# audiohacking/fp8-mps-metal

Measured on NVIDIA B200. Metric: FP8 _scaled_mm TFLOPS & M=1 GEMV/cast HBM GB/s as % roofline vs CPU ref, higher is better.
Workload: dtype f32

## Files before the change

fp8-mps-metal_b200/csrc/fp8_gemm_tcgen05.cu:

```cuda
#include <cuda.h>
#include <cstdio>
#include <mutex>
#include <type_traits>

#include "fp8_mm.cuh"
#include "fp8_async.cuh"

namespace fp8b {

constexpr int kBM = 128;
constexpr int kBK = 128;
constexpr int kUmmaK = 32;
#ifndef FP8B_EPI_WARPS
#define FP8B_EPI_WARPS 4
#endif
constexpr int kNumEpiWarps = FP8B_EPI_WARPS;
constexpr int kEpiColSplits = kNumEpiWarps / 4;
enum { kStDirect = 0, kStPeers = 1, kStTma = 2, kStWide = 3 };
template <int MODE> constexpr bool is_push() { return MODE == kStTma || MODE == kStWide; }
constexpr int kMaxDst = 8;
template <int MODE> constexpr int gemm_threads() { return 64 + 32 * kNumEpiWarps + (is_push<MODE>() ? 32 : 0); }

constexpr int kStoreBoxBytes = 128 * 128;
#ifndef FP8B_TMA_SLOTS
// ... 125 lines not shown
    uint32_t r;
    asm volatile("mov.u32 %0, %%cluster_ctarank;" : "=r"(r));
    return r;
}
__device__ __forceinline__ void cluster_sync_all() {
    asm volatile("barrier.cluster.arrive.release.aligned;" ::: "memory");
    asm volatile("barrier.cluster.wait.acquire.aligned;" ::: "memory");
}
__device__ __forceinline__ void cluster_sync_relaxed() {
    asm volatile("barrier.cluster.arrive.relaxed.aligned;" ::: "memory");
    asm volatile("barrier.cluster.wait.aligned;" ::: "memory");
}
__device__ __forceinline__ void tma_load_2d_2sm(uint32_t smem_dst, const CUtensorMap* m, uint32_t bar, int c0, int c1) {
    asm volatile("cp.async.bulk.tensor.2d.cta_group::2.shared::cluster.global.mbarrier::complete_tx::bytes [%0], [%1, {%3, %4}], [%2];"
                 :: "r"(smem_dst), "l"(reinterpret_cast<uint64_t>(m)), "r"(bar & kPeerBitMask), "r"(c0), "r"(c1) : "memory");
}
__device__ __forceinline__ void mbar_arrive_leader(uint32_t bar) {
    asm volatile("mbarrier.arrive.shared::cluster.b64 _, [%0];" :: "r"(bar & kPeerBitMask) : "memory");
}
__device__ __forceinline__ void tmem_alloc_2sm(uint32_t smem_dst, uint32_t ncols) {
    asm volatile("tcgen05.alloc.cta_group::2.sync.aligned.shared::cta.b32 [%0], %1;" :: "r"(smem_dst), "r"(ncols) : "memory");
}
__device__ __forceinline__ void tmem_relinquish_2sm() {
    asm volatile("tcgen05.relinquish_alloc_permit.cta_group::2.sync.aligned;" ::: "memory");
}
__device__ __forceinline__ void tmem_dealloc_2sm(uint32_t taddr, uint32_t ncols) {
    asm volatile("tcgen05.dealloc.cta_group::2.sync.aligned.b32 %0, %1;" :: "r"(taddr), "r"(ncols) : "memory");
}
__device__ __forceinline__ void umma_f8_2sm(uint32_t tmem_d, uint64_t adesc, uint64_t bdesc, uint32_t idesc, uint32_t accumulate) {
    asm volatile("{\n\t.reg .pred p;\n\tsetp.ne.b32 p, %4, 0;\n\t"
                 "tcgen05.mma.cta_group::2.kind::f8f6f4 [%0], %1, %2, %3, p;\n\t}"
                 :: "r"(tmem_d), "l"(adesc), "l"(bdesc), "r"(idesc), "r"(accumulate) : "memory");
}
__device__ __forceinline__ void umma_commit_2sm(uint32_t bar) {
    asm volatile("tcgen05.commit.cta_group::2.mbarrier::arrive::one.shared::cluster.multicast::cluster.b64 [%0], %1;"
                 :: "r"(bar), "h"((uint16_t)3) : "memory");
}

__device__ __forceinline__ bool elect_one() {
    uint32_t pred;
    asm volatile("{\n\t.reg .pred p;\n\telect.sync _|p, 0xFFFFFFFF;\n\tselp.u32 %0, 1, 0, p;\n\t}" : "=r"(pred));
    return pred != 0;
}

__device__ __forceinline__ uint64_t make_smem_desc(uint32_t smem_addr) {
    uint64_t d = 0;
    d |= (uint64_t)((smem_addr & 0x3FFFF) >> 4);
    d |= (uint64_t)1 << 16;
    d |= (uint64_t)(1024 >> 4) << 32;
    d |= (uint64_t)1 << 46;
    d |= (uint64_t)2 << 61;
    return d;
}

__host__ __device__ constexpr uint32_t make_idesc(int m, int n) {
    return (1u << 4) | ((uint32_t)(n >> 3) << 17) | ((uint32_t)(m >> 4) << 24);
}

__device__ __forceinline__ void stg_v4(void* p, uint32_t a, uint32_t b, uint32_t c, uint32_t d, int mc) {
    if (mc)
        asm volatile("multimem.st.weak.global.v4.f32 [%0], {%1,%2,%3,%4};"
                     :: "l"(p), "f"(__uint_as_float(a)), "f"(__uint_as_float(b)), "f"(__uint_as_float(c)),
                        "f"(__uint_as_float(d)) : "memory");
    else
        asm volatile("st.global.v4.u32 [%0], {%1,%2,%3,%4};" :: "l"(p), "r"(a), "r"(b), "r"(c), "r"(d) : "memory");
}

__device__ __forceinline__ void sts_v4(uint32_t addr, uint32_t a, uint32_t b, uint32_t c, uint32_t d) {
    asm volatile("st.shared.v4.u32 [%0], {%1,%2,%3,%4};" :: "r"(addr), "r"(a), "r"(b), "r"(c), "r"(d) : "memory");
}
__device__ __forceinline__ void lds_v4(uint32_t addr, uint32_t& a, uint32_t& b, uint32_t& c, uint32_t& d) {
    asm volatile("ld.shared.v4.u32 {%0,%1,%2,%3}, [%4];" : "=r"(a), "=r"(b), "=r"(c), "=r"(d) : "r"(addr) : "memory");
}

constexpr int kRasterGroup = 8;
struct TileCoord { int m_blk; int n0; int width; };
__device__ __forceinline__ TileCoord decode_tile(const GemmParams& p, int t, int bn) {
    TileCoord c;
    int tt = t, half = -1;
    if (t >= p.full_tiles) {
        const int u = t - p.full_tiles;
        tt = p.full_tiles + (u >> 1);
        half = u & 1;
    }
    int n_blk;
    if (p.raster_n == 2) {
        const int per_band = kRasterGroup * p.num_n_blocks;
        const int band = tt / per_band, r = tt - band * per_band;
        const int m0 = band * kRasterGroup;
        const int rows = min(kRasterGroup, p.num_m_blocks - m0);
        c.m_blk = m0 + r % rows;
        n_blk = r / rows;
    }
    else if (p.raster_n) { n_blk = tt % p.num_n_blocks; c.m_blk = tt / p.num_n_blocks; }
    else { c.m_blk = tt % p.num_m_blocks; n_blk = tt / p.num_m_blocks; }
    c.width = half < 0 ? bn : bn >> 1;
    c.n0 = n_blk * bn + (half > 0 ? c.width : 0);
    return c;
}

template <bool SBV, bool BIAS, bool SR>
__device__ __forceinline__ void epi_math32(const uint32_t (&r)[32], float sa, float sb0, float sr, const float (&sbv)[32],
                                           const float (&bv)[32], float (&v)[32]) {
#pragma unroll
    for (int j = 0; j < 32; ++j) {
        float x = __fmul_rn(__uint_as_float(r[j]), sa);
        x = __fmul_rn(x, SBV ? sbv[j] : sb0);
        if (BIAS) x = __fadd_rn(x, bv[j]);
        if (SR) x = __fmul_rn(x, sr);
        v[j] = x;
    }
}
__device__ __forceinline__ bool any_nan32(const uint32_t (&r)[32]) {
    float s0 = 0.0f, s1 = 0.0f, s2 = 0.0f, s3 = 0.0f;
#pragma unroll
    for (int j = 0; j < 32; j += 4) {
        s0 += __uint_as_float(r[j]); s1 += __uint_as_float(r[j + 1]);
        s2 += __uint_as_float(r[j + 2]); s3 += __uint_as_float(r[j + 3]);
    }
    const float s = (s0 + s1) + (s2 + s3);
    return s != s;
}

static __device__ __noinline__ void fix_nan_chunk(uint32_t* r, const uint8_t* a_row, const uint8_t* b_rows, int K, int n_left,
                                                  int a_fmt, int b_fmt) {
    for (int j = 0; j < 32 && j < n_left; ++j) {
        const float a = __uint_as_float(r[j]);
        if (a != a) r[j] = __float_as_uint(slow_dot_fmt(a_row, b_rows + (size_t)j * K, K, a_fmt, b_fmt));
    }
}
// ... 25 lines not shown
                    const float4 t = b4[j];
                    bv[4 * j] = t.x; bv[4 * j + 1] = t.y; bv[4 * j + 2] = t.z; bv[4 * j + 3] = t.w;
                }
            } else {
                const uint4* b4 = reinterpret_cast<const uint4*>(reinterpret_cast<const uint16_t*>(e.bias) + n0);
#pragma unroll
                for (int j = 0; j < 4; ++j) {
                    const uint4 t = b4[j];
                    const uint32_t w[4] = {t.x, t.y, t.z, t.w};
#pragma unroll
                    for (int i = 0; i < 4; ++i) {
                        if (e.bias_dtype == FP8B_BF16) {
                            bv[8 * j + 2 * i] = __uint_as_float(w[i] << 16);
                            bv[8 * j + 2 * i + 1] = __uint_as_float(w[i] & 0xFFFF0000u);
                        } else {
                            const float2 f = __half22float2(*reinterpret_cast<const __half2*>(&w[i]));
                            bv[8 * j + 2 * i] = f.x; bv[8 * j + 2 * i + 1] = f.y;
                        }
                    }
                }
            }
        }
    } else {
#pragma unroll
        for (int j = 0; j < 32; ++j) {
            const int n = n0 + j;
            const bool ok = n < N;
            sbv[j] = (e.sb_stride && ok) ? e.sb[n] : 0.0f;
            bv[j] = (e.bias && ok) ? epi_bias(e, n) : 0.0f;
        }
    }
}

template <int BN, int CG, int MODE = kStDirect>
__global__ void __launch_bounds__(gemm_threads<MODE>(), 1)
fp8_gemm_tcgen05_kernel(const __grid_constant__ CUtensorMap tmap_a,
                        const __grid_constant__ CUtensorMap tmap_b,
                        const __grid_constant__ typename StoreMapsOf<MODE>::type smaps,
                        const GemmParams p)
{
    using Cfg = GemmCfg<BN, CG, MODE>;
    constexpr bool PEERS = MODE == kStPeers;
#ifdef FP8B_PROFILE
    long long* const dbg = PEERS ? nullptr : p.aux;
#endif
    constexpr int kTileM = kBM * CG;
    const uint32_t cta_rank = (CG == 2) ? cluster_ctarank() : 0u;
    const bool is_leader = cta_rank == 0;
    const int worker = (CG == 2) ? (int)(blockIdx.x >> 1) : (int)blockIdx.x;
    const int num_workers = (CG == 2) ? (int)(gridDim.x >> 1) : (int)gridDim.x;
    extern __shared__ uint8_t gemm_smem_raw[];
    uint8_t* smem = reinterpret_cast<uint8_t*>((reinterpret_cast<uintptr_t>(gemm_smem_raw) + 1023) & ~(uintptr_t)1023);
    uint8_t* bar_mem = smem + Cfg::kOffBar;
    const uint32_t smem_base = smem_u32(smem);
    const uint32_t bar_base = smem_u32(bar_mem);
    auto full_bar = [&](int s) { return bar_base + 8u * s; };
    auto empty_bar = [&](int s) { return bar_base + 8u * (Cfg::kStages + s); };
    auto tfull_bar = [&](int a) { return bar_base + 8u * (2 * Cfg::kStages + a); };
    auto tempty_bar = [&](int a) { return bar_base + 8u * (2 * Cfg::kStages + 2 + a); };
    auto sfull_bar = [&](int s) { return bar_base + 8u * (2 * Cfg::kStages + 4 + s); };
    auto sfree_bar = [&](int s) { return bar_base + 8u * (2 * Cfg::kStages + 4 + Cfg::kStoreSlots + s); };
    volatile uint32_t* tmem_slot =
        reinterpret_cast<volatile uint32_t*>(bar_mem + 8 * (2 * Cfg::kStages + 4 + 2 * Cfg::kStoreSlots));
    const uint32_t stage_base = smem_base + Cfg::kOffStaging;

    const int warp = __shfl_sync(0xFFFFFFFFu, (int)(threadIdx.x >> 5), 0);
    const int lane = threadIdx.x & 31;
#ifdef FP8B_PROFILE
    if (dbg && blockIdx.x == 0 && threadIdx.x == 0) dbg[7] = clock64();
#endif

    pdl_launch_dependents();

    if (warp == kWarpTma && lane == 0) {
        tma_prefetch_desc(&tmap_a);
        tma_prefetch_desc(&tmap_b);
    }
    if (warp == kWarpMma && lane == 0) {
        for (int s = 0; s < Cfg::kStages; ++s) { mbar_init(full_bar(s), 1); mbar_init(empty_bar(s), 1); }
        for (int a = 0; a < 2; ++a) { mbar_init(tfull_bar(a), 1); mbar_init(tempty_bar(a), kNumEpiWarps * CG); }
        if (is_push<MODE>())
            for (int s = 0; s < Cfg::kStoreSlots; ++s) { mbar_init(sfull_bar(s), kNumEpiWarps); mbar_init(sfree_bar(s), 1); }
        fence_mbar_init();
        fence_proxy_async_smem();
    }
    if (warp == kWarpEpi0) {
        if (CG == 2) { tmem_alloc_2sm(smem_u32(const_cast<uint32_t*>(tmem_slot)), Cfg::kTmemCols); tmem_relinquish_2sm(); }
        else { tmem_alloc(smem_u32(const_cast<uint32_t*>(tmem_slot)), Cfg::kTmemCols); tmem_relinquish(); }
    }
    tc_fence_before();
    if (CG == 2) cluster_sync_all();
    else __syncthreads();
    tc_fence_after();
    const uint32_t tmem_base = *tmem_slot;
    pdl_wait();

    const int num_tiles = p.num_work;

    if (warp == kWarpTma) {
        {
            const bool elected = elect_one();
            int stage = 0; uint32_t phase = 0;
#ifdef FP8B_PROFILE
            int issued = 0;
#endif
            for (int tile = worker; tile < num_tiles; tile += num_workers) {
                const TileCoord tc = decode_tile(p, tile, BN);
                const int m_idx = tc.m_blk * kTileM + (int)cta_rank * kBM;
                const int n_idx = tc.n0 + (int)cta_rank * (tc.width / CG);
                for (int kb = 0; kb < p.num_k_blocks; ++kb) {
                    mbar_wait(empty_bar(stage), phase ^ 1);
                    const uint32_t a_dst = smem_base + stage * Cfg::kStageBytes;
                    if (elected) {
#ifdef FP8B_PROFILE
                        if ((p.debug & 32) && issued >= Cfg::kStages) {
                            if (is_leader) mbar_arrive(full_bar(stage));
                        } else
#endif
                        if (CG == 2) {
                            if (is_leader) mbar_arrive_expect_tx(full_bar(stage), (uint32_t)p.stage_tx * CG);
                            tma_load_2d_2sm(a_dst, &tmap_a, full_bar(stage), kb * kBK, m_idx);
                            tma_load_2d_2sm(a_dst + Cfg::kABytes, &tmap_b, full_bar(stage), kb * kBK, n_idx);
                        } else {
                            mbar_arrive_expect_tx(full_bar(stage), (uint32_t)p.stage_tx);
                            tma_load_2d(a_dst, &tmap_a, full_bar(stage), kb * kBK, m_idx);
                            tma_load_2d(a_dst + Cfg::kABytes, &tmap_b, full_bar(stage), kb * kBK, n_idx);
                        }
                    }
                    __syncwarp();
#ifdef FP8B_PROFILE
                    ++issued;
#endif
                    if (++stage == Cfg::kStages) { stage = 0; phase ^= 1; }
                }
            }
        }
    } else if (warp == kWarpMma) {
        if (is_leader) {
            constexpr uint32_t idesc = make_idesc(kTileM, BN);
            const uint32_t idesc_fmt = (((uint32_t)p.debug >> 8) & 1u) << 7 | (((uint32_t)p.debug >> 9) & 1u) << 10;
            const bool elected = elect_one();
            const uint64_t desc_a0 = make_smem_desc(smem_base);
            const uint64_t desc_b0 = make_smem_desc(smem_base + Cfg::kABytes);
            constexpr uint64_t kDescStage = (uint64_t)(Cfg::kStageBytes >> 4);
            int stage = 0; uint32_t phase = 0;
            int acc = 0; uint32_t acc_phase = 0;
            for (int tile = worker; tile < num_tiles; tile += num_workers) {
#ifdef FP8B_PROFILE
                const long long t_m0 = (dbg && blockIdx.x == 0) ? clock64() : 0;
#endif
                mbar_wait(tempty_bar(acc), acc_phase ^ 1);
                tc_fence_after();
#ifdef FP8B_PROFILE
                const long long t_m1 = (dbg && blockIdx.x == 0) ? clock64() : 0;
#endif
                const uint32_t d_tmem = tmem_base + (uint32_t)(acc * BN);
                const uint32_t idesc_t = ((tile < p.full_tiles) ? idesc : make_idesc(kTileM, BN / 2)) | idesc_fmt;
                for (int kb = 0; kb < p.num_k_blocks; ++kb) {
                    mbar_wait(full_bar(stage), phase);
                    tc_fence_after();
                    if (elected) {
                        const uint64_t adesc = desc_a0 + kDescStage * (uint64_t)stage;
                        const uint64_t bdesc = desc_b0 + kDescStage * (uint64_t)stage;
#pragma unroll
                        for (int k = 0; k < kBK / kUmmaK; ++k) {
                            if (CG == 2) umma_f8_2sm(d_tmem, adesc + 2 * k, bdesc + 2 * k, idesc_t, (uint32_t)((kb | k) != 0));
                            else umma_f8(d_tmem, adesc + 2 * k, bdesc + 2 * k, idesc_t, (uint32_t)((kb | k) != 0));
                        }
                        if (CG == 2) umma_commit_2sm(empty_bar(stage)); else umma_commit(empty_bar(stage));
                    }
                    __syncwarp();
                    if (++stage == Cfg::kStages) { stage = 0; phase ^= 1; }
                }
                if (elected) {
                    if (CG == 2) umma_commit_2sm(tfull_bar(acc)); else umma_commit(tfull_bar(acc));
#ifdef FP8B_PROFILE
                    if (dbg && blockIdx.x == 0) {
                        const int ti = (tile - worker) / num_workers;
                        if (ti < 64) { dbg[ti * 8 + 0] = t_m0; dbg[ti * 8 + 1] = t_m1; dbg[ti * 8 + 2] = clock64(); dbg[ti * 8 + 3] = 0; }
                    }
#endif
                }
                __syncwarp();
                if (++acc == 2) { acc = 0; acc_phase ^= 1; }
            }
        }
    } else if (is_push<MODE>() && warp == kWarpStore) {
        if constexpr (MODE == kStTma) {
            const bool elected = elect_one();
            const int n_dst = p.store_mc >> 8;
            const int esz = p.epi.out_dtype == FP8B_F32 ? 4 : 2;
            const int cols_per_box = 128 / esz;
            uint32_t seq = 0;
            for (int tile = worker; tile < num_tiles; tile += num_workers) {
                const TileCoord tc = decode_tile(p, tile, BN);
                const int m_idx = tc.m_blk * kTileM + (int)cta_rank * kBM;
                for (int c = 0; c < tc.width; c += cols_per_box) {
                    const int n_box = tc.n0 + c;
                    if (n_box >= p.N) break;
                    const uint32_t slot = seq % Cfg::kStoreSlots;
                    mbar_wait(sfull_bar(slot), (seq / Cfg::kStoreSlots) & 1);
                    if (elected) {
                        if (m_idx < p.M) {
                            const uint32_t src = stage_base + slot * kStoreBoxBytes;
                            for (int d = 0; d < n_dst; ++d) tma_store_2d(&smaps.m[d], src, n_box * esz, m_idx);
                        }
                        bulk_commit_group();
                        bulk_wait_group_read<kStoreInflight>();
                        if (seq >= (uint32_t)kStoreInflight) mbar_arrive(sfree_bar((seq - kStoreInflight) % Cfg::kStoreSlots));
                    }
                    __syncwarp();
                    ++seq;
                }
            }
            if (elected) bulk_wait_group_all();
            __syncwarp();
#ifdef FP8B_PROFILE
            if (dbg && blockIdx.x == 0 && lane == 0) dbg[15] = clock64();
#endif
        } else if constexpr (MODE == kStWide) {
            const bool elected = elect_one();
            const int n_dst = p.store_mc >> 8;
            constexpr int kInflight = 1;
            uint32_t seq = 0;
            for (int tile = worker; tile < num_tiles; tile += num_workers) {
                const TileCoord tc = decode_tile(p, tile, BN);
                const int m_idx = tc.m_blk * kTileM + (int)cta_rank * kBM;
                if (tc.n0 >= p.N) continue;
                const uint32_t slot = seq % Cfg::kStoreSlots;
                mbar_wait(sfull_bar(slot), (seq / Cfg::kStoreSlots) & 1);
                if (elected) {
                    if (m_idx < p.M) {
                        const uint32_t src = stage_base + slot * Cfg::kSlotBytes;
                        for (int d = 0; d < n_dst; ++d) tma_store_2d(&smaps.m[d], src, tc.n0, m_idx);
                    }
                    bulk_commit_group();
                    bulk_wait_group_read<kInflight>();
                    if (seq >= (uint32_t)kInflight) mbar_arrive(sfree_bar((seq - kInflight) % Cfg::kStoreSlots));
                }
                __syncwarp();
                ++seq;
            }
            if (elected) bulk_wait_group_all();
            __syncwarp();
        }
    } else if (is_push<MODE>()) {
        if constexpr (is_push<MODE>()) {
            constexpr bool kWide = MODE == kStWide;
            const int q = warp & 3;
            const int row_in_tile = q * 32 + lane;
            const Epi& e = p.epi;
            const float sr = e.sr ? *e.sr : 1.0f;
            const float sb0 = e.sb[0];
            const bool is_f32 = e.out_dtype == FP8B_F32;
            const int cols_per_box = kWide ? BN : 128 / (is_f32 ? 4 : 2);
            const uint32_t row_off = (uint32_t)row_in_tile * (kWide ? (uint32_t)(BN * 2) : 128u);
            uint32_t seq = 0;
            int acc = 0; uint32_t acc_phase = 0;
            if constexpr (!kWide) {
                auto run_tiles = [&](auto kind_c) {
                    constexpr int KIND = decltype(kind_c)::value;
                    constexpr bool SBV = (KIND & 1) != 0, BIAS = (KIND & 2) != 0, SR = (KIND & 4) != 0;
                    for (int tile = worker; tile < num_tiles; tile += num_workers) {
                        const TileCoord tc = decode_tile(p, tile, BN);
                        const int m_idx = tc.m_blk * kTileM + (int)cta_rank * kBM;
                        const int n_idx = tc.n0;
                        const int m = m_idx + row_in_tile;
                        const bool m_ok = m < p.M;
                        const float sa = e.sa[(size_t)(m_ok ? m : 0) * e.sa_stride];
                        const int nch = tc.width >> 5;
#ifdef FP8B_PROFILE
                        const long long t_e0 = (dbg && blockIdx.x == 0 && warp == kWarpEpi0 && lane == 0) ? clock64() : 0;
#endif
                        mbar_wait(tfull_bar(acc), acc_phase);
                        tc_fence_after();
#ifdef FP8B_PROFILE
                        const long long t_e1 = (dbg && blockIdx.x == 0 && warp == kWarpEpi0 && lane == 0) ? clock64() : 0;
#endif
                        const uint32_t t_row = tmem_base + ((uint32_t)(q * 32) << 16) + (uint32_t)(acc * BN);
                        auto release_acc = [&]() {
                            tc_fence_before();
                            __syncwarp();
                            if (lane == 0) { if (CG == 2) mbar_arrive_leader(tempty_bar(acc)); else mbar_arrive(tempty_bar(acc)); }
                        };
                        auto chunk = [&](int c0, uint32_t (&r)[32]) {
                            const int n0 = n_idx + c0;
                            const int n_box = n_idx + (c0 & ~(cols_per_box - 1));
                            if (n_box >= p.N) return;
                            const bool box_first = (c0 & (cols_per_box - 1)) == 0;
                            const bool box_last = ((c0 + 32) & (cols_per_box - 1)) == 0 || c0 + 32 == tc.width;
                            const uint32_t slot = seq % Cfg::kStoreSlots;
                            if (box_first) mbar_wait(sfree_bar(slot), ((seq / Cfg::kStoreSlots) & 1) ^ 1);
                            if (n0 < p.N) {
                                float sbv[32];
                                float bv[32];
                                if (SBV || BIAS) {
                                    if ((n0 + 32 <= p.N) && p.col_vec_ok) {
// ... 59 lines not shown
                            __syncwarp();
                            tmem_ld_wait_for(ra);
                            if (ch + 1 < nch) tmem_ld_x32(t_row + (uint32_t)((ch + 1) * 32), rb); else release_acc();
                            chunk(ch * 32, ra);
                            if (ch + 1 < nch) {
                                __syncwarp();
                                tmem_ld_wait_for(rb);
                                if (ch + 2 < nch) tmem_ld_x32(t_row + (uint32_t)((ch + 2) * 32), ra); else release_acc();
                                chunk((ch + 1) * 32, rb);
                            }
                        }
#ifdef FP8B_PROFILE
                        if (dbg && blockIdx.x == 0 && warp == kWarpEpi0 && lane == 0) {
                            const int ti = (tile - worker) / num_workers;
                            if (ti < 64) { dbg[ti * 8 + 4] = t_e0; dbg[ti * 8 + 5] = t_e1; dbg[ti * 8 + 6] = clock64(); }
                            dbg[23] = clock64();
                        }
#endif
                        if (++acc == 2) { acc = 0; acc_phase ^= 1; }
                    }
                };
                switch ((e.sb_stride ? 1 : 0) | (e.bias ? 2 : 0) | (e.sr ? 4 : 0)) {
                    case 0: run_tiles(std::integral_constant<int, 0>{}); break;
                    case 1: run_tiles(std::integral_constant<int, 1>{}); break;
                    case 2: run_tiles(std::integral_constant<int, 2>{}); break;
                    case 3: run_tiles(std::integral_constant<int, 3>{}); break;
                    case 4: run_tiles(std::integral_constant<int, 4>{}); break;
                    case 5: run_tiles(std::integral_constant<int, 5>{}); break;
                    case 6: run_tiles(std::integral_constant<int, 6>{}); break;
                    default: run_tiles(std::integral_constant<int, 7>{}); break;
                }
            } else
            for (int tile = worker; tile < num_tiles; tile += num_workers) {
                const TileCoord tc = decode_tile(p, tile, BN);
                const int m_idx = tc.m_blk * kTileM + (int)cta_rank * kBM;
                const int n_idx = tc.n0;
                const int m = m_idx + row_in_tile;
                const bool m_ok = m < p.M;
                const float sa = e.sa[(size_t)(m_ok ? m : 0) * e.sa_stride];
                mbar_wait(tfull_bar(acc), acc_phase);
                tc_fence_after();
                const uint32_t t_row = tmem_base + ((uint32_t)(q * 32) << 16) + (uint32_t)(acc * BN);
#pragma unroll 1
                for (int c0 = 0; c0 < tc.width; c0 += 32) {
                    uint32_t r[32];
                    __syncwarp();
                    tmem_ld_x32(t_row + c0, r);
                    const int n0 = n_idx + c0;
                    const int n_box = kWide ? n_idx : n_idx + (c0 & ~(cols_per_box - 1));
                    const bool box_first = kWide ? c0 == 0 : (c0 & (cols_per_box - 1)) == 0;
                    const bool box_last = kWide ? false : ((c0 + 32) & (cols_per_box - 1)) == 0;
                    const bool box_ok = n_box < p.N;
                    const bool chunk_ok = n0 < p.N;
                    float sbv[32];
                    float bv[32];
                    if (chunk_ok) load_col_params(e, n0, p.N, (n0 + 32 <= p.N) && p.col_vec_ok, sbv, bv);
                    const uint32_t slot = seq % Cfg::kStoreSlots;
                    if (box_ok && box_first) mbar_wait(sfree_bar(slot), ((seq / Cfg::kStoreSlots) & 1) ^ 1);
                    tmem_ld_wait();
                    if (c0 + 32 == tc.width) {
                        tc_fence_before();
                        __syncwarp();
                        if (lane == 0) { if (CG == 2) mbar_arrive_leader(tempty_bar(acc)); else mbar_arrive(tempty_bar(acc)); }
                    }
                    if (!box_ok) continue;
                    if (chunk_ok) {
                        float nan_probe = 0.0f;
// ... 46 lines not shown
                        fence_proxy_async_smem();
                        __syncwarp();
                        if (lane == 0) mbar_arrive(sfull_bar(slot));
                        ++seq;
                    }
                }
                if (++acc == 2) { acc = 0; acc_phase ^= 1; }
            }
        }
    } else {
        const int q = warp & 3;
        const int col_part = (warp - kWarpEpi0) >> 2;
        const int row_in_tile = q * 32 + lane;
        const Epi& e = p.epi;
        const float sr = e.sr ? *e.sr : 1.0f;
        const float sb0 = e.sb[0];
        long long peer_delta[8];
        const int peer_world = PEERS ? (p.store_mc >> 8) : 0;
        if (PEERS) {
#pragma unroll
            for (int r = 0; r < 8; ++r) peer_delta[r] = r < peer_world ? p.aux[r] : 0;
        }
        auto store16 = [&](void* ptr, uint32_t a, uint32_t b, uint32_t c, uint32_t d) {
            if (PEERS) {
#pragma unroll
                for (int r = 0; r < 8; ++r)
                    if (r < peer_world) stg_v4(reinterpret_cast<uint8_t*>(ptr) + peer_delta[r], a, b, c, d, 0);
            } else {
                stg_v4(ptr, a, b, c, d, p.store_mc & 1);
            }
        };
        int acc = 0; uint32_t acc_phase = 0;
        for (int tile = worker; tile < num_tiles; tile += num_workers) {
            const TileCoord tc = decode_tile(p, tile, BN);
            const int m_idx = tc.m_blk * kTileM + (int)cta_rank * kBM;
            const int n_idx = tc.n0;
            const int cols_per_warp = tc.width / kEpiColSplits;
            const int m = m_idx + row_in_tile;
            const bool m_ok = m < p.M;
            const float sa = e.sa[(size_t)(m_ok ? m : 0) * e.sa_stride];
#ifdef FP8B_PROFILE
            const long long t_e0 = (dbg && blockIdx.x == 0 && warp == kWarpEpi0 && lane == 0) ? clock64() : 0;
#endif
            mbar_wait(tfull_bar(acc), acc_phase);
            tc_fence_after();
#ifdef FP8B_PROFILE
            const long long t_e1 = (dbg && blockIdx.x == 0 && warp == kWarpEpi0 && lane == 0) ? clock64() : 0;
#endif
            const uint32_t t_row = tmem_base + ((uint32_t)(q * 32) << 16) + (uint32_t)(acc * BN);
#pragma unroll 1
            for (int c0 = col_part * cols_per_warp; c0 < (col_part + 1) * cols_per_warp; c0 += 32) {
                uint32_t r[32];
                __syncwarp();
                tmem_ld_x32(t_row + c0, r);
                const int n0 = n_idx + c0;
                const bool full_chunk = (n0 + 32 <= p.N) && p.col_vec_ok;
                float sbv[32];
                float bv[32];
                if (full_chunk) load_col_params(e, n0, p.N, true, sbv, bv);
                tmem_ld_wait();
                if (c0 + 32 == (col_part + 1) * cols_per_warp) {
                    tc_fence_before();
                    __syncwarp();
                    if (lane == 0) { if (CG == 2) mbar_arrive_leader(tempty_bar(acc)); else mbar_arrive(tempty_bar(acc)); }
                }
                if (n0 >= p.N) continue;
                if (FP8B_DBG(p, 2)) continue;
// ... 472 lines not shown

bool tcgen05_supported(const MMArgs& a)
{
    return a.M >= 1 && a.N >= 1 && a.K >= 16 && (a.K % 16 == 0) && aligned(a.A, 16) && aligned(a.B, 16);
}

static bool tma_store_ok(const MMArgs& a, void* const* dsts, int n_dst)
{
    const size_t esz = dtype_size(a.out_dtype);
    if ((a.ldc * esz) % 16 != 0) return false;
    if (((size_t)a.N * esz) % 16 != 0) return false;
    for (int d = 0; d < n_dst; ++d)
        if (!dsts[d] || !aligned(dsts[d], 16)) return false;
    return true;
}

static void fill_signal(StoreMaps& sm, const MMArgs& a)
{
    sm.n_sig = 0; sm.cta_counter = nullptr; sm.epoch = 0;
    for (int d = 0; d < kMaxDst; ++d) sm.sig[d] = nullptr;
    if (!a.sig) return;
    sm.n_sig = a.store_mc >> 8;
    for (int d = 0; d < sm.n_sig; ++d) sm.sig[d] = reinterpret_cast<unsigned long long*>(a.sig->flags[d]);
    sm.cta_counter = a.sig->cta_counter;
    sm.epoch = a.sig->epoch;
}

int launch_peer_wait(const uint64_t* flags, int world, int rank, uint64_t epoch, cudaStream_t st)
{
    return launch_ex(fp8_peer_wait_kernel, dim3(1), dim3(32), 0, st, 1, 1, true,
                     reinterpret_cast<const unsigned long long*>(flags), world, rank, (unsigned long long)epoch);
}

template <int BN, int CG, int MODE = kStDirect>
static int launch_tcgen05_cfg(const MMArgs& a)
{
    using Cfg = GemmCfg<BN, CG, MODE>;
    static std::atomic<int> attr_done[64];
    if (int rc = ensure_max_smem(fp8_gemm_tcgen05_kernel<BN, CG, MODE>, Cfg::kSmemBytes, attr_done)) return rc;

    CUtensorMap tmap_a, tmap_b;
    const int a_box_rows = a.M < kBM ? ((a.M + 7) / 8) * 8 : kBM;
    if (!encode_operand_map(&tmap_a, a.A, a.M, a.K, a_box_rows)) return FP8B_ERR_CUDA;
    if (!encode_operand_map(&tmap_b, a.B, a.N, a.K, Cfg::kBRows)) return FP8B_ERR_CUDA;

    const size_t esz = dtype_size(a.out_dtype);
    GemmParams p;
    p.A = a.A; p.B = a.B; p.M = a.M; p.N = a.N; p.K = a.K;
    p.num_m_blocks = (a.M + kBM * CG - 1) / (kBM * CG);
    p.num_n_blocks = (a.N + BN - 1) / BN;
    p.num_k_blocks = (a.K + kBK - 1) / kBK;
    {
        const int forced_r = tune(kTuneGemmRaster, 0);
        const size_t b_bytes = (size_t)a.N * a.K, a_bytes = (size_t)a.M * a.K;
        const bool n_fast = b_bytes <= ((size_t)48 << 20) || b_bytes <= a_bytes;
        const bool grouped = a_bytes > ((size_t)32 << 20) && b_bytes > ((size_t)32 << 20) && p.num_m_blocks > kRasterGroup;
        p.raster_n = forced_r ? (forced_r == 3 ? 2 : forced_r == 2) : grouped ? 2 : n_fast;
    }
    const int tiles_all = p.num_m_blocks * p.num_n_blocks;
    const int workers_cap = device_info().sm_count / CG;
    p.full_tiles = tiles_all;
    p.num_work = tiles_all;
    {
        const int rem = tiles_all % workers_cap;
        bool can_split = (BN % 64 == 0) && ((BN / 2 / CG) % 8 == 0) && tiles_all > workers_cap;
        if (MODE == kStTma) can_split = can_split && ((BN / 2) * esz) % 128 == 0;
        if (MODE == kStWide) can_split = false;
#ifdef FP8B_PROFILE
        can_split = can_split && !(tune_int("FP8B_GEMM_DEBUG", 0) & 8);
#endif
        if (can_split && rem > 0 && 2 * rem <= workers_cap) {
            p.full_tiles = tiles_all - rem;
            p.num_work = tiles_all + rem;
        }
    }
    p.epi = make_epi(a);
    p.vec_store_ok = aligned(a.C, 16) && ((a.ldc * esz) % 16 == 0);
    p.col_vec_ok = (a.sb_len == 1 || aligned(a.sb, 16)) && (!a.bias || aligned(a.bias, 16));
    p.debug = (a.a_fmt ? 0x100 : 0) | (a.b_fmt ? 0x200 : 0);
    p.store_mc = a.store_mc;
    p.aux = nullptr;
    p.stage_tx = a_box_rows * kBK + Cfg::kBBytes;
    typename StoreMapsOf<MODE>::type smaps;
    if constexpr (MODE == kStPeers) {
        p.aux = static_cast<long long*>(a.ws);
    } else if constexpr (MODE == kStTma) {
        const int n_dst = a.store_mc >> 8;
        void* const* dsts = static_cast<void* const*>(a.ws);
        void* self[1] = {a.C};
        if (!dsts) dsts = self;
        if (n_dst < 1 || n_dst > kMaxDst || !tma_store_ok(a, dsts, n_dst)) return FP8B_ERR_UNSUPPORTED;
        for (int d = 0; d < n_dst; ++d)
            if (!get_tensor_map(&smaps.m[d], dsts[d], (uint64_t)a.M, (uint64_t)a.N * esz, (uint64_t)a.ldc * esz, 128, 128))
                return FP8B_ERR_CUDA;
        for (int d = n_dst; d < kMaxDst; ++d) smaps.m[d] = smaps.m[0];
        fill_signal(smaps, a);
    } else if constexpr (MODE == kStWide) {
        const int n_dst = a.store_mc >> 8;
        void* const* dsts = static_cast<void* const*>(a.ws);
        void* self[1] = {a.C};
        if (!dsts) dsts = self;
        if (esz != 2 || n_dst < 1 || n_dst > kMaxDst || !tma_store_ok(a, dsts, n_dst)) return FP8B_ERR_UNSUPPORTED;
        for (int d = 0; d < n_dst; ++d)
            if (!get_tensor_map(&smaps.m[d], dsts[d], (uint64_t)a.M, (uint64_t)a.N, (uint64_t)a.ldc * 2, 128, BN, 2, false))
                return FP8B_ERR_CUDA;
        for (int d = n_dst; d < kMaxDst; ++d) smaps.m[d] = smaps.m[0];
        fill_signal(smaps, a);
    } else {
        smaps.unused = 0;
    }
#ifdef FP8B_PROFILE
    if constexpr (MODE != kStPeers) {
        p.debug |= tune_int("FP8B_GEMM_DEBUG", 0) & 0xFF;
        if (p.debug & 16) {
            static long long* dbuf = nullptr;
            if (!dbuf) cudaMalloc(&dbuf, 64 * 8 * sizeof(long long));
            cudaMemset(dbuf, 0, 64 * 8 * sizeof(long long));
            p.aux = dbuf;
        }
    }
#endif
    if (!is_push<MODE>() && a.store_mc && !(p.vec_store_ok && p.col_vec_ok && a.N % 32 == 0)) return FP8B_ERR_UNSUPPORTED;

    const int tiles = p.num_work;
    const int workers_max = workers_cap;
    const int workers = tiles < workers_max ? tiles : workers_max;

    cudaLaunchConfig_t cfg = {};
    cfg.gridDim = dim3(workers * CG, 1, 1);
    cfg.blockDim = dim3(gemm_threads<MODE>(), 1, 1);
    cfg.dynamicSmemBytes = Cfg::kSmemBytes;
    cfg.stream = a.st;
    cudaLaunchAttribute attr[3];
    int nattr = 0;
    if (CG > 1) {
        attr[nattr].id = cudaLaunchAttributeClusterDimension;
        attr[nattr].val.clusterDim.x = CG; attr[nattr].val.clusterDim.y = 1; attr[nattr].val.clusterDim.z = 1;
        ++nattr;
    }
    if (g_opt_pdl.load(std::memory_order_relaxed)) {
        attr[nattr].id = cudaLaunchAttributeProgrammaticStreamSerialization;
        attr[nattr].val.programmaticStreamSerializationAllowed = 1;
        ++nattr;
    }
    cfg.attrs = attr;
    cfg.numAttrs = nattr;
    cudaError_t e = cudaLaunchKernelEx(&cfg, fp8_gemm_tcgen05_kernel<BN, CG, MODE>, tmap_a, tmap_b, smaps, p);
    if (e != cudaSuccess) return cuda_fail(e);
#ifdef FP8B_PROFILE
    if (MODE != kStPeers && p.aux) {
        long long h[64 * 8];
        cudaDeviceSynchronize();
        cudaMemcpy(h, p.aux, sizeof(h), cudaMemcpyDeviceToHost);
        printf("CTA 0: kernel entry -> first MMA wait %lld cycles; last epilogue end -> stores complete %lld; -> CTA end %lld\n",
               h[0] - h[7], h[15] ? h[15] - h[23] : 0, h[31] - (h[15] ? h[15] : h[23]));
        printf("tile | mma: wait_tempty  issue+run (of which waiting for TMA) | epi: wait_tfull  drain+store | epi_end - mma_end\n");
        for (int t = 0; t < 64 && h[t * 8 + 2]; ++t)
            printf("%4d | %8lld %8lld (%8lld) | %8lld %8lld | %8lld   (mma start %lld)\n", t, h[t * 8 + 1] - h[t * 8 + 0],
                   h[t * 8 + 2] - h[t * 8 + 1], h[t * 8 + 3], h[t * 8 + 5] - h[t * 8 + 4], h[t * 8 + 6] - h[t * 8 + 5],
                   h[t * 8 + 6] - h[t * 8 + 2], h[t * 8 + 0] - h[0]);
    }
#endif
    return after_launch();
}

template <int S>
static int launch_splitk(const MMArgs& a)
{
    static std::atomic<int> attr_done[64];
    if (int rc = ensure_max_smem(fp8_gemm_splitk_kernel<S>, kSkSmemBytes, attr_done)) return rc;
    const int a_box_rows = a.M < kBM ? ((a.M + 7) / 8) * 8 : kBM;
    CUtensorMap tmap_a, tmap_b;
    if (!encode_operand_map(&tmap_a, a.A, a.M, a.K, a_box_rows)) return FP8B_ERR_CUDA;
    if (!encode_operand_map(&tmap_b, a.B, a.N, a.K, 128)) return FP8B_ERR_CUDA;
    const size_t esz = dtype_size(a.out_dtype);
    SplitKParams p;
    p.A = a.A; p.B = a.B; p.M = a.M; p.N = a.N; p.K = a.K;
    p.num_n_blocks = (a.N + 127) / 128;
    p.num_k_blocks = (a.K + kBK - 1) / kBK;
    p.stage_tx = a_box_rows * kBK + 128 * kBK;
// ... 67 lines not shown
    const long tiles128 = (long)((a.M + kBM - 1) / kBM) * ((a.N + 127) / 128);
    if (!pairs_only && (tiles128 <= sms || (tiles128 <= 2L * sms && a.K <= 1024))) return 2;
    if (a.M > 128 && a.N > 128) {
        const long mt = (a.M + 255) / 256;
        const int pairs = sms / 2;
        const double kf = (double)a.K / 3072.0;
        auto cost = [&](int width) {
            const double t3072 = width == 256 ? 10.5 : width == 192 ? 9.3 : 8.65;
            const long tiles = mt * ((a.N + width - 1) / width);
            return (1.5 + kf * (t3072 - 1.5)) * (double)((tiles + pairs - 1) / pairs);
        };
        int cfg = 3;
        double best = cost(256);
        if (cost(192) < best) { best = cost(192); cfg = 5; }
        if (cost(128) < best) { best = cost(128); cfg = 4; }
        return cfg;
    }
    const long t_256 = (long)((a.M + kBM - 1) / kBM) * ((a.N + 255) / 256);
    return (a.N > 128 && t_256 >= 2L * sms) ? 1 : 2;
}

int launch_gemm_tcgen05(const MMArgs& a)
{
    if (!tcgen05_supported(a)) return FP8B_ERR_UNSUPPORTED;
    const int forced = tune(kTuneGemmCfg, 0);
    const int mode = a.store_mc & 0xFF;
    int cfg = forced ? forced : pick_tile_cfg(a, mode == 2);
    if (mode == 0 && !forced) {
        const int split = pick_split_k(a);
        if (split == 4) return launch_splitk<4>(a);
        if (split == 2) return launch_splitk<2>(a);
    }
    if (!forced && mode == 3 && (a.store_mc >> 8) > 1 && (cfg == 3 || cfg == 5)) cfg = 4;
    if (mode == 2) {
        if ((a.store_mc >> 8) < 2 || (a.store_mc >> 8) > 8 || !a.ws) return FP8B_ERR_INVALID;
        switch (cfg) {
            case 3: return launch_tcgen05_cfg<256, 2, kStPeers>(a);
            case 4: return launch_tcgen05_cfg<128, 2, kStPeers>(a);
            case 5: return launch_tcgen05_cfg<192, 2, kStPeers>(a);
            default: return FP8B_ERR_UNSUPPORTED;
        }
    }
    if (mode == 3) {
        const int st = tune(kTuneGemmStore, 0);
        const bool wide = dtype_size(a.out_dtype) == 2 && (st == 3 || (st != 4 && kPushWideDefault && (a.store_mc >> 8) > 1));
        if (wide) {
            switch (cfg) {
                case 1: return launch_tcgen05_cfg<256, 1, kStWide>(a);
                case 3: return launch_tcgen05_cfg<256, 2, kStWide>(a);
                case 4: return launch_tcgen05_cfg<128, 2, kStWide>(a);
                case 5: return launch_tcgen05_cfg<192, 2, kStWide>(a);
                default: return launch_tcgen05_cfg<128, 1, kStWide>(a);
            }
        }
        switch (cfg) {
            case 1: return launch_tcgen05_cfg<256, 1, kStTma>(a);
            case 3: return launch_tcgen05_cfg<256, 2, kStTma>(a);
            case 4: return launch_tcgen05_cfg<128, 2, kStTma>(a);
            case 5: return launch_tcgen05_cfg<192, 2, kStTma>(a);
            default: return launch_tcgen05_cfg<128, 1, kStTma>(a);
        }
    }
    if (mode == 0 && tune(kTuneGemmStore, kDefaultGemmStore) == 2) {
        void* self[1] = {a.C};
        if (tma_store_ok(a, self, 1)) {
            MMArgs t = a;
            t.store_mc = 3 | (1 << 8);
            t.ws = nullptr;
            switch (cfg) {
                case 1: return launch_tcgen05_cfg<256, 1, kStTma>(t);
                case 3: return launch_tcgen05_cfg<256, 2, kStTma>(t);
                case 4: return launch_tcgen05_cfg<128, 2, kStTma>(t);
                case 5: return launch_tcgen05_cfg<192, 2, kStTma>(t);
                default: return launch_tcgen05_cfg<128, 1, kStTma>(t);
            }
        }
    }
    switch (cfg) {
        case 1: return launch_tcgen05_cfg<256, 1>(a);
        case 3: return launch_tcgen05_cfg<256, 2>(a);
        case 4: return launch_tcgen05_cfg<128, 2>(a);
        case 5: return launch_tcgen05_cfg<192, 2>(a);
        default: return launch_tcgen05_cfg<128, 1>(a);
    }
}

}
```

Measured before the change: 2807.

## Add opt-in 4-CTA cluster config multicasting A tiles across two CTA pairs

Adds a PPC=2 kernel variant in which two 2-SM CTA pairs form a 4-CTA cluster. Each pair loads half of the shared A tile and multicasts it to both pairs, which roughly halves A global/L2 traffic; the pairs split the N range of a wider tile. Stage-release commits now go to all four CTAs, and the grid is capped by the occupancy query for 4-CTA clusters. The raster heuristic is also changed so the small-B N-fast rule applies only to multi-destination stores, which alters raster order for some single-destination GEMMs. The new cluster config is only reached when forced through the tuning knob.

```diff
diff --git a/fp8-mps-metal_b200/csrc/fp8_gemm_tcgen05.cu b/fp8-mps-metal_b200/csrc/fp8_gemm_tcgen05.cu
--- a/fp8-mps-metal_b200/csrc/fp8_gemm_tcgen05.cu
+++ b/fp8-mps-metal_b200/csrc/fp8_gemm_tcgen05.cu
@@ -181,9 +181,16 @@
                  "tcgen05.mma.cta_group::2.kind::f8f6f4 [%0], %1, %2, %3, p;\n\t}"
                  :: "r"(tmem_d), "l"(adesc), "l"(bdesc), "r"(idesc), "r"(accumulate) : "memory");
 }
-__device__ __forceinline__ void umma_commit_2sm(uint32_t bar) {
+__device__ __forceinline__ void umma_commit_2sm(uint32_t bar, uint16_t cta_mask) {
     asm volatile("tcgen05.commit.cta_group::2.mbarrier::arrive::one.shared::cluster.multicast::cluster.b64 [%0], %1;"
-                 :: "r"(bar), "h"((uint16_t)3) : "memory");
+                 :: "r"(bar), "h"(cta_mask) : "memory");
+}
+__device__ __forceinline__ void tma_load_2d_2sm_mc(uint32_t smem_dst, const CUtensorMap* m, uint32_t bar, int c0, int c1,
+                                                   uint16_t cta_mask) {
+    asm volatile("cp.async.bulk.tensor.2d.shared::cluster.global.tile.mbarrier::complete_tx::bytes.multicast::cluster.cta_group::2"
+                 " [%0], [%1, {%3, %4}], [%2], %5;"
+                 :: "r"(smem_dst), "l"(reinterpret_cast<uint64_t>(m)), "r"(bar & kPeerBitMask), "r"(c0), "r"(c1), "h"(cta_mask)
+                 : "memory");
 }
 
 __device__ __forceinline__ bool elect_one() {
@@ -245,6 +252,12 @@
     else { c.m_blk = tt % p.num_m_blocks; n_blk = tt / p.num_m_blocks; }
     c.width = half < 0 ? bn : bn >> 1;
     c.n0 = n_blk * bn + (half > 0 ? c.width : 0);
+    return c;
+}
+template <int BN, int PPC>
+__device__ __forceinline__ TileCoord pair_tile(const GemmParams& p, int t, int pair) {
+    TileCoord c = decode_tile(p, t, BN * PPC);
+    if (PPC > 1) { c.width /= PPC; c.n0 += pair * c.width; }
     return c;
 }
 
@@ -336,7 +349,7 @@
     }
 }
 
-template <int BN, int CG, int MODE = kStDirect>
+template <int BN, int CG, int MODE = kStDirect, int PPC = 1>
 __global__ void __launch_bounds__(gemm_threads<MODE>(), 1)
 fp8_gemm_tcgen05_kernel(const __grid_constant__ CUtensorMap tmap_a,
                         const __grid_constant__ CUtensorMap tmap_b,
@@ -345,14 +358,18 @@
 {
     using Cfg = GemmCfg<BN, CG, MODE>;
     constexpr bool PEERS = MODE == kStPeers;
+    static_assert(PPC == 1 || (PPC == 2 && CG == 2), "clusters of two pairs are built from CTA pairs");
 #ifdef FP8B_PROFILE
     long long* const dbg = PEERS ? nullptr : p.aux;
 #endif
     constexpr int kTileM = kBM * CG;
-    const uint32_t cta_rank = (CG == 2) ? cluster_ctarank() : 0u;
+    constexpr int kCluster = CG * PPC;
+    const uint32_t cl_rank = (kCluster > 1) ? cluster_ctarank() : 0u;
+    const uint32_t cta_rank = cl_rank & (uint32_t)(CG - 1);
+    const int pair = (int)(cl_rank >> 1);
     const bool is_leader = cta_rank == 0;
-    const int worker = (CG == 2) ? (int)(blockIdx.x >> 1) : (int)blockIdx.x;
-    const int num_workers = (CG == 2) ? (int)(gridDim.x >> 1) : (int)gridDim.x;
+    const int worker = (int)blockIdx.x / kCluster;
+    const int num_workers = (int)gridDim.x / kCluster;
     extern __shared__ uint8_t gemm_smem_raw[];
     uint8_t* smem = reinterpret_cast<uint8_t*>((reinterpret_cast<uintptr_t>(gemm_smem_raw) + 1023) & ~(uintptr_t)1023);
     uint8_t* bar_mem = smem + Cfg::kOffBar;
@@ -381,7 +398,7 @@
         tma_prefetch_desc(&tmap_b);
     }
     if (warp == kWarpMma && lane == 0) {
-        for (int s = 0; s < Cfg::kStages; ++s) { mbar_init(full_bar(s), 1); mbar_init(empty_bar(s), 1); }
+        for (int s = 0; s < Cfg::kStages; ++s) { mbar_init(full_bar(s), 1); mbar_init(empty_bar(s), PPC); }
         for (int a = 0; a < 2; ++a) { mbar_init(tfull_bar(a), 1); mbar_init(tempty_bar(a), kNumEpiWarps * CG); }
         if (is_push<MODE>())
             for (int s = 0; s < Cfg::kStoreSlots; ++s) { mbar_init(sfull_bar(s), kNumEpiWarps); mbar_init(sfree_bar(s), 1); }
@@ -409,9 +426,11 @@
             int issued = 0;
 #endif
             for (int tile = worker; tile < num_tiles; tile += num_workers) {
-                const TileCoord tc = decode_tile(p, tile, BN);
+                const TileCoord tc = pair_tile<BN, PPC>(p, tile, pair);
                 const int m_idx = tc.m_blk * kTileM + (int)cta_rank * kBM;
                 const int n_idx = tc.n0 + (int)cta_rank * (tc.width / CG);
+                constexpr uint32_t kAHalf = kBM / 2 * kBK;
+                const uint16_t a_mask = (uint16_t)((1u << cl_rank) | (1u << (cl_rank ^ 2u)));
                 for (int kb = 0; kb < p.num_k_blocks; ++kb) {
                     mbar_wait(empty_bar(stage), phase ^ 1);
                     const uint32_t a_dst = smem_base + stage * Cfg::kStageBytes;
@@ -423,7 +442,11 @@
 #endif
                         if (CG == 2) {
                             if (is_leader) mbar_arrive_expect_tx(full_bar(stage), (uint32_t)p.stage_tx * CG);
-                            tma_load_2d_2sm(a_dst, &tmap_a, full_bar(stage), kb * kBK, m_idx);
+                            if (PPC == 2)
+                                tma_load_2d_2sm_mc(a_dst + (uint32_t)pair * kAHalf, &tmap_a, full_bar(stage), kb * kBK,
+                                                   m_idx + pair * (kBM / 2), a_mask);
+                            else
+                                tma_load_2d_2sm(a_dst, &tmap_a, full_bar(stage), kb * kBK, m_idx);
                             tma_load_2d_2sm(a_dst + Cfg::kABytes, &tmap_b, full_bar(stage), kb * kBK, n_idx);
                         } else {
                             mbar_arrive_expect_tx(full_bar(stage), (uint32_t)p.stage_tx);
@@ -447,6 +470,8 @@
             const uint64_t desc_a0 = make_smem_desc(smem_base);
             const uint64_t desc_b0 = make_smem_desc(smem_base + Cfg::kABytes);
             constexpr uint64_t kDescStage = (uint64_t)(Cfg::kStageBytes >> 4);
+            constexpr uint16_t kCommitAll = (uint16_t)((1u << kCluster) - 1u);
+            const uint16_t pair_mask = (uint16_t)(3u << (2 * pair));
             int stage = 0; uint32_t phase = 0;
             int acc = 0; uint32_t acc_phase = 0;
             for (int tile = worker; tile < num_tiles; tile += num_workers) {
@@ -471,13 +496,13 @@
                             if (CG == 2) umma_f8_2sm(d_tmem, adesc + 2 * k, bdesc + 2 * k, idesc_t, (uint32_t)((kb | k) != 0));
                             else umma_f8(d_tmem, adesc + 2 * k, bdesc + 2 * k, idesc_t, (uint32_t)((kb | k) != 0));
                         }
-                        if (CG == 2) umma_commit_2sm(empty_bar(stage)); else umma_commit(empty_bar(stage));
+                        if (CG == 2) umma_commit_2sm(empty_bar(stage), kCommitAll); else umma_commit(empty_bar(stage));
                     }
                     __syncwarp();
                     if (++stage == Cfg::kStages) { stage = 0; phase ^= 1; }
                 }
                 if (elected) {
-                    if (CG == 2) umma_commit_2sm(tfull_bar(acc)); else umma_commit(tfull_bar(acc));
+                    if (CG == 2) umma_commit_2sm(tfull_bar(acc), pair_mask); else umma_commit(tfull_bar(acc));
 #ifdef FP8B_PROFILE
                     if (dbg && blockIdx.x == 0) {
                         const int ti = (tile - worker) / num_workers;
@@ -497,7 +522,7 @@
             const int cols_per_box = 128 / esz;
             uint32_t seq = 0;
             for (int tile = worker; tile < num_tiles; tile += num_workers) {
-                const TileCoord tc = decode_tile(p, tile, BN);
+                const TileCoord tc = pair_tile<BN, PPC>(p, tile, pair);
                 const int m_idx = tc.m_blk * kTileM + (int)cta_rank * kBM;
                 for (int c = 0; c < tc.width; c += cols_per_box) {
                     const int n_box = tc.n0 + c;
@@ -528,7 +553,7 @@
             constexpr int kInflight = 1;
             uint32_t seq = 0;
             for (int tile = worker; tile < num_tiles; tile += num_workers) {
-                const TileCoord tc = decode_tile(p, tile, BN);
+                const TileCoord tc = pair_tile<BN, PPC>(p, tile, pair);
                 const int m_idx = tc.m_blk * kTileM + (int)cta_rank * kBM;
                 if (tc.n0 >= p.N) continue;
                 const uint32_t slot = seq % Cfg::kStoreSlots;
@@ -566,7 +591,7 @@
                     constexpr int KIND = decltype(kind_c)::value;
                     constexpr bool SBV = (KIND & 1) != 0, BIAS = (KIND & 2) != 0, SR = (KIND & 4) != 0;
                     for (int tile = worker; tile < num_tiles; tile += num_workers) {
-                        const TileCoord tc = decode_tile(p, tile, BN);
+                        const TileCoord tc = pair_tile<BN, PPC>(p, tile, pair);
                         const int m_idx = tc.m_blk * kTileM + (int)cta_rank * kBM;
                         const int n_idx = tc.n0;
                         const int m = m_idx + row_in_tile;
@@ -692,7 +717,7 @@
                 }
             } else
             for (int tile = worker; tile < num_tiles; tile += num_workers) {
-                const TileCoord tc = decode_tile(p, tile, BN);
+                const TileCoord tc = pair_tile<BN, PPC>(p, tile, pair);
                 const int m_idx = tc.m_blk * kTileM + (int)cta_rank * kBM;
                 const int n_idx = tc.n0;
                 const int m = m_idx + row_in_tile;
@@ -805,7 +830,7 @@
         };
         int acc = 0; uint32_t acc_phase = 0;
         for (int tile = worker; tile < num_tiles; tile += num_workers) {
-            const TileCoord tc = decode_tile(p, tile, BN);
+            const TileCoord tc = pair_tile<BN, PPC>(p, tile, pair);
             const int m_idx = tc.m_blk * kTileM + (int)cta_rank * kBM;
             const int n_idx = tc.n0;
             const int cols_per_warp = tc.width / kEpiColSplits;
@@ -1344,33 +1369,67 @@
                      reinterpret_cast<const unsigned long long*>(flags), world, rank, (unsigned long long)epoch);
 }
 
-template <int BN, int CG, int MODE = kStDirect>
+template <int BN, int MODE>
+static int max_active_clusters4()
+{
+    using Cfg = GemmCfg<BN, 2, MODE>;
+    static std::atomic<int> cached[64];
+    int dev = 0;
+    if (cudaGetDevice(&dev) != cudaSuccess || dev < 0 || dev >= 64) return 0;
+    int n = cached[dev].load(std::memory_order_acquire);
+    if (n > 0) return n;
+    cudaLaunchConfig_t cfg = {};
+    cfg.gridDim = dim3(4 * (unsigned)device_info().sm_count, 1, 1);
+    cfg.blockDim = dim3(gemm_threads<MODE>(), 1, 1);
+    cfg.dynamicSmemBytes = Cfg::kSmemBytes;
+    cudaLaunchAttribute attr;
+    attr.id = cudaLaunchAttributeClusterDimension;
+    attr.val.clusterDim.x = 4; attr.val.clusterDim.y = 1; attr.val.clusterDim.z = 1;
+    cfg.attrs = &attr;
+    cfg.numAttrs = 1;
+    if (cudaOccupancyMaxActiveClusters(&n, fp8_gemm_tcgen05_kernel<BN, 2, MODE, 2>, &cfg) != cudaSuccess) {
+        (void)cudaGetLastError();
+        return 0;
+    }
+    cached[dev].store(n, std::memory_order_release);
+    return n;
+}
+
+template <int BN, int CG, int MODE = kStDirect, int PPC = 1>
 static int launch_tcgen05_cfg(const MMArgs& a)
 {
     using Cfg = GemmCfg<BN, CG, MODE>;
+    constexpr int kCluster = CG * PPC;
     static std::atomic<int> attr_done[64];
-    if (int rc = ensure_max_smem(fp8_gemm_tcgen05_kernel<BN, CG, MODE>, Cfg::kSmemBytes, attr_done)) return rc;
+    if (int rc = ensure_max_smem(fp8_gemm_tcgen05_kernel<BN, CG, MODE, PPC>, Cfg::kSmemBytes, attr_done)) return rc;
+    int workers_cap = device_info().sm_count / CG;
+    if (PPC == 2) {
+        workers_cap = max_active_clusters4<BN, MODE>();
+        if (workers_cap <= 0) return FP8B_ERR_UNSUPPORTED;
+    }
 
     CUtensorMap tmap_a, tmap_b;
+    if (PPC == 2 && a.M < kBM) return FP8B_ERR_UNSUPPORTED;
     const int a_box_rows = a.M < kBM ? ((a.M + 7) / 8) * 8 : kBM;
-    if (!encode_operand_map(&tmap_a, a.A, a.M, a.K, a_box_rows)) return FP8B_ERR_CUDA;
+    if (!encode_operand_map(&tmap_a, a.A, a.M, a.K, PPC == 2 ? kBM / 2 : a_box_rows)) return FP8B_ERR_CUDA;
     if (!encode_operand_map(&tmap_b, a.B, a.N, a.K, Cfg::kBRows)) return FP8B_ERR_CUDA;
 
     const size_t esz = dtype_size(a.out_dtype);
     GemmParams p;
     p.A = a.A; p.B = a.B; p.M = a.M; p.N = a.N; p.K = a.K;
     p.num_m_blocks = (a.M + kBM * CG - 1) / (kBM * CG);
-    p.num_n_blocks = (a.N + BN - 1) / BN;
+    p.num_n_blocks = (a.N + BN * PPC - 1) / (BN * PPC);
+
     p.num_k_blocks = (a.K + kBK - 1) / kBK;
     {
         const int forced_r = tune(kTuneGemmRaster, 0);
         const size_t b_bytes = (size_t)a.N * a.K, a_bytes = (size_t)a.M * a.K;
-        const bool n_fast = b_bytes <= ((size_t)48 << 20) || b_bytes <= a_bytes;
+        const bool one_dst = is_push<MODE>() ? (a.store_mc >> 8) == 1 : a.store_mc == 0;
+        const bool n_fast = b_bytes <= a_bytes || (!one_dst && b_bytes <= ((size_t)48 << 20));
         const bool grouped = a_bytes > ((size_t)32 << 20) && b_bytes > ((size_t)32 << 20) && p.num_m_blocks > kRasterGroup;
         p.raster_n = forced_r ? (forced_r == 3 ? 2 : forced_r == 2) : grouped ? 2 : n_fast;
     }
     const int tiles_all = p.num_m_blocks * p.num_n_blocks;
-    const int workers_cap = device_info().sm_count / CG;
     p.full_tiles = tiles_all;
     p.num_work = tiles_all;
     {
@@ -1435,19 +1494,18 @@
     if (!is_push<MODE>() && a.store_mc && !(p.vec_store_ok && p.col_vec_ok && a.N % 32 == 0)) return FP8B_ERR_UNSUPPORTED;
 
     const int tiles = p.num_work;
-    const int workers_max = workers_cap;
-    const int workers = tiles < workers_max ? tiles : workers_max;
+    const int workers = tiles < workers_cap ? tiles : workers_cap;
 
     cudaLaunchConfig_t cfg = {};
-    cfg.gridDim = dim3(workers * CG, 1, 1);
+    cfg.gridDim = dim3(workers * kCluster, 1, 1);
     cfg.blockDim = dim3(gemm_threads<MODE>(), 1, 1);
     cfg.dynamicSmemBytes = Cfg::kSmemBytes;
     cfg.stream = a.st;
     cudaLaunchAttribute attr[3];
     int nattr = 0;
-    if (CG > 1) {
+    if (kCluster > 1) {
         attr[nattr].id = cudaLaunchAttributeClusterDimension;
-        attr[nattr].val.clusterDim.x = CG; attr[nattr].val.clusterDim.y = 1; attr[nattr].val.clusterDim.z = 1;
+        attr[nattr].val.clusterDim.x = kCluster; attr[nattr].val.clusterDim.y = 1; attr[nattr].val.clusterDim.z = 1;
         ++nattr;
     }
     if (g_opt_pdl.load(std::memory_order_relaxed)) {
@@ -1457,7 +1515,7 @@
     }
     cfg.attrs = attr;
     cfg.numAttrs = nattr;
-    cudaError_t e = cudaLaunchKernelEx(&cfg, fp8_gemm_tcgen05_kernel<BN, CG, MODE>, tmap_a, tmap_b, smaps, p);
+    cudaError_t e = cudaLaunchKernelEx(&cfg, fp8_gemm_tcgen05_kernel<BN, CG, MODE, PPC>, tmap_a, tmap_b, smaps, p);
     if (e != cudaSuccess) return cuda_fail(e);
 #ifdef FP8B_PROFILE
     if (MODE != kStPeers && p.aux) {
@@ -1591,6 +1649,7 @@
         if (split == 2) return launch_splitk<2>(a);
     }
     if (!forced && mode == 3 && (a.store_mc >> 8) > 1 && (cfg == 3 || cfg == 5)) cfg = 4;
+    if (cfg == 6 && (mode != 0 || a.M < kBM)) cfg = 3;
     if (mode == 2) {
         if ((a.store_mc >> 8) < 2 || (a.store_mc >> 8) > 8 || !a.ws) return FP8B_ERR_INVALID;
         switch (cfg) {
@@ -1629,6 +1688,7 @@
             switch (cfg) {
                 case 1: return launch_tcgen05_cfg<256, 1, kStTma>(t);
                 case 3: return launch_tcgen05_cfg<256, 2, kStTma>(t);
+                case 6: return launch_tcgen05_cfg<256, 2, kStTma, 2>(t);
                 case 4: return launch_tcgen05_cfg<128, 2, kStTma>(t);
                 case 5: return launch_tcgen05_cfg<192, 2, kStTma>(t);
                 default: return launch_tcgen05_cfg<128, 1, kStTma>(t);
@@ -1637,7 +1697,7 @@
     }
     switch (cfg) {
         case 1: return launch_tcgen05_cfg<256, 1>(a);
-        case 3: return launch_tcgen05_cfg<256, 2>(a);
+        case 3: case 6: return launch_tcgen05_cfg<256, 2>(a);
         case 4: return launch_tcgen05_cfg<128, 2>(a);
         case 5: return launch_tcgen05_cfg<192, 2>(a);
         default: return launch_tcgen05_cfg<128, 1>(a);
```

Result: faster. 2872, median of 6 (+2.3%).
